# siesta-tool/SequenceDetectionQueryExecutor

Measured on NVIDIA B200. Metric: events scanned/sec (/detection verification), higher is better.
Workload: dtype int32

## Files before the change

sequencedetectionqueryexecutor_b200/csrc/detect.cu:

```cuda
#include <algorithm>
#include <cstdio>
#include <type_traits>
#include <cstdlib>
#include <cstring>
#include <vector>

#include "detect_common.cuh"

namespace siesta {

template <int W, int R, int NF, bool SMEM_RUNS>
struct WarpSmem {
    static constexpr int NE = ROWS_OF(W);
    static constexpr size_t famvv_off = 0;
    static constexpr size_t famvv_bytes = SMEM_RUNS ? sizeof(unsigned long long) * NF * 32 : 0;
    static constexpr size_t rmask_off = famvv_off + famvv_bytes;
    static constexpr size_t rmask_bytes = SMEM_RUNS ? sizeof(typename MaskOps<W>::T) * R * 32 : 0;
    typedef typename std::conditional<W == 1, uint16_t, uint32_t>::type small_t;
    static constexpr size_t small_off = rmask_off + rmask_bytes;
    static constexpr size_t small_bytes = sizeof(small_t) * NE * 32;
    static constexpr size_t rmeta_off = (small_off + small_bytes + 15) & ~(size_t)15;
    static constexpr size_t rmeta_bytes = SMEM_RUNS ? sizeof(uint32_t) * R * 32 : 0;
    static constexpr size_t bytes_off = rmeta_off + rmeta_bytes;
    static constexpr size_t bytes_bytes = SMEM_RUNS ? (size_t)(R + 3 * NF) * 32 : 0;
// ... 775 lines not shown
}

__global__ void set_tail_kernel(int64_t* occ_off, int64_t n_tr, int64_t n_occ, int64_t* ev_off, int64_t n_ev, RebaseOffsets base) {
    occ_off[n_tr] = n_occ + base.occ;
    ev_off[n_occ] = n_ev + base.ev;
}

namespace {

struct DevBuf {
    void* p = nullptr;
    Ctx* c = nullptr;
    explicit DevBuf(Ctx* ctx) : c(ctx) {}
    DevBuf(const DevBuf&) = delete;
    ~DevBuf() { if (p) dev_arena_free(c, p); }
    int alloc(size_t bytes) {
        if (p) { dev_arena_free(c, p); p = nullptr; }
        p = dev_arena_alloc(c, bytes);
        return p ? SIESTA_OK : SIESTA_E_NOMEM;
    }
    template <class T> T* as() const { return reinterpret_cast<T*>(p); }
    void* release() { void* q = p; p = nullptr; return q; }
};

struct View {
    void* p;
    template <class T> T* as() const { return reinterpret_cast<T*>(p); }
};

template <int W, int R, int NF, bool SMEM_RUNS, int MODE>
int launch_detect(const Ctx* ctx, cudaStream_t stream, DetectParams P, const DevNfa& nfa) {
    typedef WarpSmem<W, R, NF, SMEM_RUNS> L;
    const bool needs_aux = MODE == FAST_NK && (P.flags & SIESTA_F_RETURN_ALL) != 0;
    int nt = NT;
    if (const char* env = std::getenv("SIESTA_K1_THREADS")) {
        const int v = std::atoi(env);
        if (v >= 32 && v <= NT_MAX && v % 32 == 0) nt = v;
    }
    const size_t smem = L::total(needs_aux) * (nt / 32);
    auto kern = detect_kernel<W, R, NF, SMEM_RUNS, MODE>;
    SIESTA_CUDA_OK(cudaFuncSetAttribute(kern, cudaFuncAttributeMaxDynamicSharedMemorySize, (int)smem));
    if (const char* env = std::getenv("SIESTA_K1_CARVEOUT")) {
        const int v = std::atoi(env);
        if (v >= 0 && v <= 100) SIESTA_CUDA_OK(cudaFuncSetAttribute(kern, cudaFuncAttributePreferredSharedMemoryCarveout, v));
    }
    int per_sm = 0;
    SIESTA_CUDA_OK(cudaOccupancyMaxActiveBlocksPerMultiprocessor(&per_sm, kern, nt, smem));
    if (per_sm < 1) per_sm = 1;
    const int64_t n_tiles = (P.n_work + 31) / 32;
    const int64_t ctas_needed = (n_tiles + nt / 32 - 1) / (nt / 32);
    if (const char* env = std::getenv("SIESTA_K1_CTAS_PER_SM")) {
        const int v = std::atoi(env);
        if (v >= 1 && v < per_sm) per_sm = v;
    }
    int grid = (int)std::min<int64_t>(ctas_needed, (int64_t)ctx->sm_count * per_sm);
    if (P.n_work_dev) grid = std::min(grid, ctx->sm_count * 2);
    if (grid < 1) grid = 1;
    kern<<<grid, nt, smem, stream>>>(P, nfa);
    SIESTA_LAUNCHED();
    SIESTA_CUDA_OK(cudaGetLastError());
    return SIESTA_OK;
}

}

struct DetectPending {
    Log* log = nullptr;
    cudaStream_t stream = nullptr;
    int64_t n = 0;
    uint32_t flags = 0;
    RebaseOffsets base{0, 0, 0};
    const int64_t* d_cand = nullptr;
    DetectParams P;
    size_t n_blk = 0;
    unsigned long long *d_blk = nullptr, *d_top = nullptr, *d_counters = nullptr;
    int64_t* d_err = nullptr;
    int64_t* d_unsup = nullptr;
    int unsup_slot = 7;
    void* work = nullptr;
    int uniform_k = 0;
    cudaEvent_t ev0 = nullptr, evd = nullptr;
    unsigned long long* h_cnt = nullptr;
    const uint16_t* d_lut = nullptr;
    const uint4* d_nkp_lut = nullptr;
};

static unsigned long long* pinned_counters_get(Ctx* c) {
    std::lock_guard<std::mutex> g(c->arena_mu);
    if (c->pinned_counters.empty()) {
        void* slab = nullptr;
        if (cudaHostAlloc(&slab, 32 * 128, cudaHostAllocDefault) != cudaSuccess) return nullptr;
        c->pinned_slabs.push_back(slab);
        for (int i = 0; i < 32; ++i) c->pinned_counters.push_back(reinterpret_cast<unsigned long long*>(reinterpret_cast<char*>(slab) + 128 * i));
    }
    unsigned long long* p = c->pinned_counters.back();
    c->pinned_counters.pop_back();
    return p;
}
static void pinned_counters_put(Ctx* c, unsigned long long* p) {
    if (!p) return;
    std::lock_guard<std::mutex> g(c->arena_mu);
    c->pinned_counters.push_back(p);
}

static void pending_discard(DetectPending* q) {
    if (!q) return;
    if (q->work) dev_arena_free(q->log->ctx, q->work);
    if (q->ev0) cudaEventDestroy(q->ev0);
    if (q->evd) cudaEventDestroy(q->evd);
    pinned_counters_put(q->log->ctx, q->h_cnt);
    delete q;
}

int detect_device_finish_impl(DetectPending* q, siesta_dev_matches* out);

int detect_device_begin_impl(Log* log, const siesta_nfa* nfa, const int64_t* d_cand, int64_t n_cand, uint32_t flags,
                             cudaStream_t stream, RebaseOffsets base, DetectPending** pending, const DetectPending* sibling) {
    *pending = nullptr;
    base.trace += log->first_trace;
    DevNfa dn;
    int rc = validate_nfa(nfa, flags, &dn);
    if (rc != SIESTA_OK) return rc;
    const Ctx* ctx = log->ctx;
    SIESTA_CUDA_OK(cudaSetDevice(ctx->device));
    if (!stream) stream = ctx->stream;
    const int64_t n = d_cand ? n_cand : log->n_traces;
    const bool return_all = (flags & SIESTA_F_RETURN_ALL) != 0;
    const bool all_cols = (flags & SIESTA_F_NO_EVENT_COLUMNS) == 0;

    std::vector<uint16_t> lut;
    int needs_ts = 0, n_positive = 0;
    build_lut(nfa, dn, log->n_activities, flags, lut, &needs_ts, &n_positive);

    const int64_t wide = std::min<int64_t>(log->n_events, n * 64);
    const int64_t cap_occ = return_all ? wide : n;
    const int64_t cap_ev = (!return_all && !dn.any_kleene) ? n * std::max(1, n_positive) : wide;

    DevBuf work(log->ctx);
    const size_t nn = (size_t)std::max<int64_t>(n, 1);
    size_t w_off = 0;
    auto carve = [&w_off](size_t bytes) {
        const size_t at = w_off;
        w_off += (bytes + 255) & ~(size_t)255;
        return at;
    };
    NkwProgram prog;
    const int nkw_space = nkw_build(dn, flags, &prog);
    std::vector<uint16_t> sigs;
    for (size_t a = 0; a < lut.size(); ++a) {
        const uint16_t sg = lut[a] & 0xFFu;
        if (sg && std::find(sigs.begin(), sigs.end(), sg) == sigs.end()) sigs.push_back(sg);
    }
    const bool use_nkp = nkw_space != NKW_NONE && (!needs_ts || return_all) && log->act_valid && log->n_activities <= 255 && !sigs.empty() && sigs.size() <= 7 &&
                         (reinterpret_cast<uintptr_t>(log->d_act) & 31u) == 0 && std::getenv("SIESTA_K1_NO_NKP") == nullptr;
    const size_t reg2 = use_nkp ? (size_t)std::max<int64_t>(cap_ev, n * (int64_t)std::max(1, n_positive)) : 0;
    const bool use_long = dn.fast_class == FAST_NK && std::getenv("SIESTA_K1_NO_LONG") == nullptr;
    const int64_t cap_long = use_long ? std::min<int64_t>(log->n_events, (int64_t)1 << 21) : 0;
    const size_t long_pool = use_long ? (size_t)std::min<int64_t>(std::max<int64_t>(log->n_events * 64, (int64_t)1 << 20), (int64_t)256 << 20) : 0;
    const size_t n_blk = (nn + GT - 1) / GT;
    const size_t o_ovf2 = use_nkp ? carve(nn * 8) : 0;
    const size_t o_unsup = carve((size_t)SIESTA_MAX_UNSUPPORTED * 8);
    const size_t o_unsup2 = use_long ? carve((size_t)SIESTA_MAX_UNSUPPORTED * 8) : 0;
    const size_t o_pool = carve(long_pool);
    const size_t o_nlut = use_nkp ? carve((size_t)(log->n_activities + 1) * 16) : 0;
    const size_t o_lut = carve(lut.size() * sizeof(uint16_t)), o_nocc = carve(nn * 4), o_stage = carve(nn * 8),
                 o_stage_occ = carve(return_all ? nn * 8 : 0), o_counters = carve(32 * 8), o_err = carve(nn * 8), o_ovf = carve(nn * 8),
                 o_blk = carve(n_blk * 3 * 8), o_top = carve(((n_blk + 1023) / 1024) * 3 * 8), o_occ_nev = carve(return_all ? ((size_t)(cap_occ + cap_long) + (use_nkp ? nn : 0)) * 4 : 0), o_pos = carve(((size_t)cap_ev + reg2 + (size_t)cap_long) * 4);
    size_t o_rank = 0, o_act = 0, o_ts = 0;
    if (all_cols) {
        o_rank = carve(((size_t)cap_ev + reg2 + (size_t)cap_long) * 4);
        o_act = carve(((size_t)cap_ev + reg2 + (size_t)cap_long) * 4);
        o_ts = carve(((size_t)cap_ev + reg2 + (size_t)cap_long) * 8);
    }
    if ((rc = work.alloc(w_off))) return rc;
    char* wb = work.as<char>();
    const View b_lut{wb + o_lut}, b_nocc{wb + o_nocc}, b_stage{wb + o_stage}, b_stage_occ{wb + o_stage_occ},
        b_counters{wb + o_counters}, b_err{wb + o_err}, b_ovf{wb + o_ovf}, b_blk{wb + o_blk}, s_occ_nev{wb + o_occ_nev},
        s_ev_pos{wb + o_pos}, s_ev_rank{all_cols ? wb + o_rank : nullptr}, s_ev_act{all_cols ? wb + o_act : nullptr},
        s_ev_ts{all_cols ? wb + o_ts : nullptr};

    cudaEvent_t ev0 = nullptr, evd = nullptr;
    SIESTA_CUDA_OK(cudaEventCreate(&ev0));
    SIESTA_CUDA_OK(cudaEventCreate(&evd));
    unsigned long long* h_cnt = nullptr;
    const uint4* d_nkp_lut = nullptr;
    struct BeginGuard {
        cudaEvent_t &a, &b;
        unsigned long long*& h;
        Ctx* c;
        bool armed;
        ~BeginGuard() {
            if (!armed) return;
            if (a) cudaEventDestroy(a);
            if (b) cudaEventDestroy(b);
            pinned_counters_put(c, h);
        }
    } begin_guard{ev0, evd, h_cnt, log->ctx, true};
    if (!sibling) SIESTA_CUDA_OK(cudaMemcpyAsync(b_lut.p, lut.data(), lut.size() * sizeof(uint16_t), cudaMemcpyHostToDevice, stream));
    SIESTA_CUDA_OK(cudaMemsetAsync(b_counters.p, 0, 256, stream));
    SIESTA_CUDA_OK(cudaMemsetAsync(b_blk.p, 0, n_blk * 3 * 8, stream));
    SIESTA_CUDA_OK(cudaEventRecord(ev0, stream));

    DetectParams P;
    std::memset(&P, 0, sizeof(P));
    P.trace_off = log->d_trace_off;
    P.act = log->d_act;
    P.ts_ms = log->d_ts_ms;
    P.cand = d_cand;
    P.work = nullptr;
    P.n_work = n;
    P.lut = sibling ? sibling->d_lut : b_lut.as<uint16_t>();
    P.n_act = log->n_activities;
    P.n_events = log->n_events;
    P.alpha_mode = !log->act_valid ? 2 : (log->n_activities <= 32 ? 0 : (log->n_activities <= 64 ? 1 : 2));
    std::memset(P.relrev, 0, sizeof(P.relrev));
    std::memset(P.cls_word, 0, sizeof(P.cls_word));
    std::memset(P.cls_act, 0, sizeof(P.cls_act));
    P.n_planes = 1;
    if (P.alpha_mode != 2) {
        int K = 0;
        for (size_t a = 0; a < lut.size(); ++a) K += lut[a] != 0;
        if (K > 7) P.alpha_mode = 2;
        else {
            int c = 0;
            for (size_t a = 0; a < lut.size(); ++a) {
                if (!lut[a]) continue;
                ++c;
                P.cls_word[c] = lut[a];
                P.cls_act[c] = (int32_t)a;
                for (int p = 0; p < 3; ++p)
                    if ((c >> p) & 1) P.relrev[p][a >> 5] |= 0x80000000u >> (a & 31);
            }
            P.n_planes = K <= 1 ? 1 : (K <= 3 ? 2 : 3);
        }
    }
    P.vec_ok = (reinterpret_cast<uintptr_t>(log->d_act) & 15u) == 0 ? 1 : 0;
    P.flags = flags;
    P.needs_ts = needs_ts;
    P.d_cnt = b_nocc.as<uint32_t>();
    P.d_stage = b_stage.as<int64_t>();
    P.d_stage_occ = b_stage_occ.as<int64_t>();
    P.s_occ_nev = s_occ_nev.as<int32_t>();
    P.s_ev_pos = s_ev_pos.as<int32_t>();
    P.s_ev_rank = s_ev_rank.as<int32_t>();
    P.s_ev_act = s_ev_act.as<int32_t>();
    P.s_ev_ts = s_ev_ts.as<int64_t>();
    P.cap_occ = cap_occ;
    P.cap_ev = cap_ev;
    P.counters = b_counters.as<unsigned long long>();
    P.err_list = b_err.as<int64_t>();
    P.ovf_list = b_ovf.as<int64_t>();
    P.blk_sums = b_blk.as<unsigned long long>();
    P.n_blk = (int64_t)n_blk;

    P.ovf_slot = 4;
    P.tile_slot = 16;
    h_cnt = pinned_counters_get(log->ctx);
    if (!h_cnt) {
        set_error("cudaHostAlloc (counters) failed");
        return SIESTA_E_NOMEM;
    }
    std::memset(h_cnt, 0, 128);
    if (n > 0) {
        if (use_nkp) {
            DetectParams N = P;
            N.ovf_list = reinterpret_cast<int64_t*>(wb + o_ovf2);
            N.ovf_slot = 13;
            N.tile_slot = 18;
            N.fix_ev = cap_ev;
            N.fix_np = std::max(1, n_positive);
            N.fix_occ = return_all ? cap_occ + cap_long : -1;
            std::vector<uint32_t> nlut((size_t)(log->n_activities + 1) * 4, 0u);
            std::memset(N.cls_word, 0, sizeof(N.cls_word));
            for (int a = 0; a <= log->n_activities; ++a) {
                const uint16_t sg = a < log->n_activities ? (lut[a] & 0xFFu) : 0;
                int c = 0;
                if (sg) {
                    c = (int)(std::find(sigs.begin(), sigs.end(), sg) - sigs.begin()) + 1;
                    N.cls_word[c] = sg;
                }
                nlut[4 * a + 0] = (nkw_space == NKW_RAW || c) ? 2u : 1u;
                for (int p = 0; p < 3; ++p) nlut[4 * a + 1 + p] = (c >> p) & 1;
            }
            if (sibling && sibling->d_nkp_lut) N.nkp_lut = sibling->d_nkp_lut;
            else {
                SIESTA_CUDA_OK(cudaMemcpyAsync(wb + o_nlut, nlut.data(), nlut.size() * 4, cudaMemcpyHostToDevice, stream));
                N.nkp_lut = reinterpret_cast<const uint4*>(wb + o_nlut);
            }
            d_nkp_lut = N.nkp_lut;
            N.n_planes = sigs.size() <= 1 ? 1 : (sigs.size() <= 3 ? 2 : 3);
            std::memset(N.st_inv, 0, sizeof(N.st_inv));
            std::memset(N.st_single, 0, sizeof(N.st_single));
            for (int k = 0; k < nfa->n_states; ++k) {
                int n_own = 0, c_own = 0;
                for (int c = 1; c <= (int)sigs.size(); ++c)
                    if (sigs[(size_t)c - 1] & (1u << k)) {
                        ++n_own;
                        c_own = c;
                    }
                if (n_own == 1) {
                    N.st_single[k] = 1;
                    for (int p = 0; p < 3; ++p) N.st_inv[k][p] = ((c_own >> p) & 1) ? 0u : 0xFFFFFFFFu;
                }
            }
            if ((rc = launch_nkp(ctx, stream, N, prog, nkw_space))) return rc;
            P.work = N.ovf_list;
            P.n_work_dev = b_counters.as<unsigned long long>() + 13;
        }
        if (dn.fast_class == FAST_FK2) rc = launch_detect<1, 0, 0, false, FAST_FK2>(ctx, stream, P, dn);
        else if (dn.fast_class == FAST_NK) rc = launch_detect<1, 0, 0, false, FAST_NK>(ctx, stream, P, dn);
        else if (dn.fast_class == FAST_NP1) rc = launch_detect<1, 0, 0, false, FAST_NP1>(ctx, stream, P, dn);
        else rc = launch_detect<1, 16, 16, true, FAST_NONE>(ctx, stream, P, dn);
        if (rc) return rc;
        SIESTA_CUDA_OK(cudaEventRecord(evd, stream));
        DetectParams Q = P;
        Q.work = b_ovf.as<int64_t>();
        Q.n_work_dev = b_counters.as<unsigned long long>() + 4;
        Q.ovf_list = reinterpret_cast<int64_t*>(wb + o_unsup);
        Q.ovf_cap = SIESTA_MAX_UNSUPPORTED;
        Q.ovf_slot = 7;
        Q.tile_slot = 17;
        if (dn.fast_class == FAST_FK2) rc = launch_detect<2, 0, 0, false, FAST_FK2>(ctx, stream, Q, dn);
        else if (dn.fast_class == FAST_NK) rc = launch_detect<2, 0, 0, false, FAST_NK>(ctx, stream, Q, dn);
        else if (dn.fast_class == FAST_NP1) rc = launch_detect<2, 0, 0, false, FAST_NP1>(ctx, stream, Q, dn);
        else rc = launch_detect<2, 1024, 128, false, FAST_NONE>(ctx, stream, Q, dn);
        if (rc) return rc;
        if (use_long) {
            LongParams LQ;
            std::memset(&LQ, 0, sizeof(LQ));
            LQ.work = reinterpret_cast<const int64_t*>(wb + o_unsup);
            LQ.n_work_dev = b_counters.as<unsigned long long>() + 7;
            LQ.work_cap = SIESTA_MAX_UNSUPPORTED;
            LQ.pool = wb + o_pool;
            LQ.pool_bytes = long_pool;
            LQ.ev_base = (int64_t)cap_ev + (int64_t)reg2;
            LQ.ev_cap = cap_long;
            LQ.occ_base = cap_occ;
            LQ.occ_cap = cap_long;
            LQ.unsup = reinterpret_cast<int64_t*>(wb + o_unsup2);
            LQ.unsup_cap = SIESTA_MAX_UNSUPPORTED;
            LQ.n_positive = std::max(1, n_positive);
            detect_long_kernel<<<ctx->sm_count * 2, 128, 0, stream>>>(P, LQ, dn);
            SIESTA_LAUNCHED();
            SIESTA_CUDA_OK(cudaGetLastError());
        }
        if (!sibling) SIESTA_CUDA_OK(cudaMemcpyAsync(h_cnt, b_counters.p, 128, cudaMemcpyDeviceToHost, stream));
    }
    DetectPending* q = new DetectPending();
    q->log = log;
    q->stream = stream;
    q->n = n;
    q->flags = flags;
    q->base = base;
    q->d_cand = d_cand;
    q->P = P;
    q->n_blk = n_blk;
    q->d_blk = b_blk.as<unsigned long long>();
    q->d_top = reinterpret_cast<unsigned long long*>(wb + o_top);
    q->d_counters = b_counters.as<unsigned long long>();
    q->d_err = b_err.as<int64_t>();
    q->d_unsup = reinterpret_cast<int64_t*>(wb + (use_long ? o_unsup2 : o_unsup));
    q->unsup_slot = use_long ? 14 : 7;
    q->work = work.release();
    q->uniform_k = (!return_all && !dn.any_kleene) ? std::max(1, n_positive) : 0;
    q->ev0 = ev0;
    q->evd = evd;
    q->h_cnt = h_cnt;
    q->d_lut = P.lut;
    q->d_nkp_lut = d_nkp_lut;
    begin_guard.armed = false;
    *pending = q;
    return SIESTA_OK;
}

int detect_device_finish_impl(DetectPending* q, siesta_dev_matches* out) {
    std::memset(out, 0, sizeof(*out));
    struct Guard {
        DetectPending* q;
        ~Guard() { pending_discard(q); }
    } guard{q};
    Log* log = q->log;
    const Ctx* ctx = log->ctx;
    SIESTA_CUDA_OK(cudaSetDevice(ctx->device));
    cudaStream_t stream = q->stream;
    const int64_t n = q->n;
    const uint32_t flags = q->flags;
    const bool return_all = (flags & SIESTA_F_RETURN_ALL) != 0;
    const bool all_cols = (flags & SIESTA_F_NO_EVENT_COLUMNS) == 0;
    const RebaseOffsets base = q->base;
    const int64_t* d_cand = q->d_cand;
    const DetectParams& P = q->P;
    const size_t n_blk = q->n_blk;
    unsigned long long* h_cnt = q->h_cnt;
    cudaEvent_t ev0 = q->ev0, evd = q->evd, ev1;
    int rc = SIESTA_OK;
    SIESTA_CUDA_OK(cudaStreamSynchronize(stream));
    if (n > 0) {
        if (h_cnt[7] > SIESTA_MAX_UNSUPPORTED || h_cnt[q->unsup_slot] > SIESTA_MAX_UNSUPPORTED) {
            set_error(std::to_string(h_cnt[7]) + " traces exceed the engine limits (64 pattern-relevant events, 1024 live runs or "
                      "65536 events per trace); at most " + std::to_string(SIESTA_MAX_UNSUPPORTED) + " are listed per request");
            return SIESTA_E_UNSUPPORTED;
        }
        if (h_cnt[5] > 0) {
            set_error("internal: occurrence staging overflow");
            return SIESTA_E_NOMEM;
        }
    }
    SIESTA_CUDA_OK(cudaEventCreate(&ev1));
    struct EvGuard {
        cudaEvent_t e;
        ~EvGuard() { cudaEventDestroy(e); }
    } ev1_guard{ev1};
#ifdef SIESTA_PHASE_TIMING
    fprintf(stderr, "[siesta phase timing] warp-cycles: filter %llu engine %llu output %llu\n", h_cnt[8], h_cnt[9], h_cnt[10]);
#endif
    const int64_t n_occ = (int64_t)h_cnt[0], n_ev = (int64_t)h_cnt[1], n_tr = (int64_t)h_cnt[6], n_err = (int64_t)h_cnt[3];
    const int64_t n_unsup = n > 0 ? (int64_t)h_cnt[q->unsup_slot] : 0;

    DevBuf fin(log->ctx);
    size_t f_off = 0;
    auto fcarve = [&f_off](size_t bytes) {
        const size_t at = f_off;
        f_off += (bytes + 255) & ~(size_t)255;
        return at;
    };
    const size_t q_trace = fcarve((size_t)n_tr * 8), q_occ = fcarve((size_t)(n_tr + 1) * 8), q_evoff = fcarve((size_t)(n_occ + 1) * 8),
                 q_pos = fcarve((size_t)n_ev * 4), q_err = fcarve((size_t)n_err * 8);
    size_t q_rank = 0, q_act = 0, q_ts = 0;
    if (all_cols) {
        q_rank = fcarve((size_t)n_ev * 4);
        q_act = fcarve((size_t)n_ev * 4);
        q_ts = fcarve((size_t)n_ev * 8);
    }
    const size_t q_unsup = fcarve((size_t)n_unsup * 8);
    if ((rc = fin.alloc(f_off))) return rc;
    char* fb = fin.as<char>();
    const View f_unsup{fb + q_unsup};
    const View f_trace{fb + q_trace}, f_occ_off{fb + q_occ}, f_ev_off{fb + q_evoff}, f_pos{fb + q_pos}, f_err{fb + q_err},
        f_rank{all_cols ? fb + q_rank : nullptr}, f_act{all_cols ? fb + q_act : nullptr}, f_ts{all_cols ? fb + q_ts : nullptr};

    if (n > 0) {
        GatherParams G;
        std::memset(&G, 0, sizeof(G));
        G.cand = d_cand;
        G.base = base;
        G.n = n;
        G.d_cnt = P.d_cnt;
        G.d_stage = P.d_stage;
        G.d_stage_occ = return_all ? P.d_stage_occ : nullptr;
        G.n_blk = (int64_t)n_blk;
        G.blk = q->d_blk;
        G.n_chunks = (int64_t)((n_blk + 1023) / 1024);
// ... 467 lines not shown
```

sequencedetectionqueryexecutor_b200/csrc/detect_common.cuh:

```cuda
#pragma once
#include "detect_fast.cuh"

namespace siesta {

constexpr int NT = 128;
constexpr int NT_MAX = 128;
#define ROWS_OF(W) ((W) == 1 ? 24 : 64)

struct DetectParams {
    const int64_t* trace_off;
    const int32_t* act;
    const int64_t* ts_ms;
    const int64_t* cand;
    const int64_t* work;
    int64_t n_work;
    const unsigned long long* n_work_dev;
    int32_t ovf_slot;
    int32_t tile_slot;
    const uint16_t* lut;
    uint32_t relrev[3][2];
    uint16_t cls_word[8];
    int32_t cls_act[8];
    int32_t n_planes;
    int64_t n_events;
    int32_t alpha_mode;
    int32_t vec_ok;
    int32_t n_act;
    uint32_t flags;
    int32_t needs_ts;
    uint32_t* d_cnt;
    int64_t* d_stage;
    int64_t* d_stage_occ;
    int32_t* s_occ_nev;
    int32_t* s_ev_pos;
    int32_t* s_ev_rank;
    int32_t* s_ev_act;
    int64_t* s_ev_ts;
    int64_t cap_occ, cap_ev;
    int64_t fix_ev;
    int32_t fix_np;
    int64_t fix_occ;
    uint32_t st_inv[SIESTA_MAX_STATES][3];
    uint8_t st_single[SIESTA_MAX_STATES];
    const uint4* nkp_lut;
    int32_t tile_batch;
    unsigned long long* counters;
    unsigned long long* blk_sums;
    int64_t n_blk;
    int64_t* err_list;
    int64_t* ovf_list;
    int64_t ovf_cap;
};

__device__ __forceinline__ long long shfl_i64(long long v, int src) {
    int lo = __shfl_sync(0xffffffffu, (int)(v & 0xffffffffll), src);
    int hi = __shfl_sync(0xffffffffu, (int)(v >> 32), src);
    return ((long long)hi << 32) | (unsigned int)lo;
}

enum { ST_NONE = 0, ST_MATCH = 1, ST_ERR = 2, ST_OVF = 3 };

__device__ __forceinline__ void load_sectors(const DetectParams& P, long long e, long long o0, long long o1, int4 (&v)[8]) {
#pragma unroll
    for (int q = 0; q < 4; ++q) {
        const long long c = e + 8 * q;
        if (c >= o1) {
            v[2 * q] = v[2 * q + 1] = make_int4(-1, -1, -1, -1);
        } else if (P.vec_ok && c + 8 <= P.n_events) {
            v[2 * q] = __ldg(reinterpret_cast<const int4*>(P.act + c));
            v[2 * q + 1] = __ldg(reinterpret_cast<const int4*>(P.act + c + 4));
        } else {
            int a[8];
#pragma unroll
            for (int i = 0; i < 8; ++i) a[i] = (c + i < o1 && c + i >= o0) ? __ldg(P.act + c + i) : -1;
            v[2 * q] = make_int4(a[0], a[1], a[2], a[3]);
            v[2 * q + 1] = make_int4(a[4], a[5], a[6], a[7]);
        }
    }
}
__device__ __forceinline__ void load_sectors_vec(const DetectParams& P, long long e, long long o1, int4 (&v)[8]) {
    const int none = P.n_act;
#pragma unroll
    for (int q = 0; q < 4; ++q) {
        const long long c = e + 8 * q;
        if (c >= o1) {
            v[2 * q] = v[2 * q + 1] = make_int4(none, none, none, none);
        } else {
            asm volatile("ld.global.nc.v8.s32 {%0,%1,%2,%3,%4,%5,%6,%7}, [%8];"
                         : "=r"(v[2 * q].x), "=r"(v[2 * q].y), "=r"(v[2 * q].z), "=r"(v[2 * q].w), "=r"(v[2 * q + 1].x),
                           "=r"(v[2 * q + 1].y), "=r"(v[2 * q + 1].z), "=r"(v[2 * q + 1].w)
                         : "l"(P.act + c));
        }
    }
}

__device__ __forceinline__ void load_quarter(const DetectParams& P, long long e, long long o1, int4 (&v)[4]) {
    const int none = P.n_act;
#pragma unroll
    for (int q = 0; q < 2; ++q) {
        const long long c = e + 8 * q;
        if (c >= o1) {
            v[2 * q] = v[2 * q + 1] = make_int4(none, none, none, none);
        } else {
            asm volatile("ld.global.nc.v8.s32 {%0,%1,%2,%3,%4,%5,%6,%7}, [%8];"
                         : "=r"(v[2 * q].x), "=r"(v[2 * q].y), "=r"(v[2 * q].z), "=r"(v[2 * q].w), "=r"(v[2 * q + 1].x),
                           "=r"(v[2 * q + 1].y), "=r"(v[2 * q + 1].z), "=r"(v[2 * q + 1].w)
                         : "l"(P.act + c));
        }
    }
}

__device__ __forceinline__ uint32_t rel_push32(uint32_t pend, uint32_t relrev, int a) {
    uint32_t t;
    asm("shl.b32 %0, %1, %2;" : "=r"(t) : "r"(relrev), "r"(a));
    return __funnelshift_r(t, pend, 31);
}
__device__ __forceinline__ uint32_t rel_push64(uint32_t pend, uint32_t relrev_a, uint32_t relrev_b, int a) {
    uint32_t t;
    const uint32_t w = ((unsigned)a < 32u) ? relrev_a : (((unsigned)a < 64u) ? relrev_b : 0u);
    asm("shl.b32 %0, %1, %2;" : "=r"(t) : "r"(w), "r"(a & 31));
    return __funnelshift_r(t, pend, 31);
}

template <int NPL, bool WIDE>
__device__ __forceinline__ void scan_block(const DetectParams& P, const int4 (&v)[8], uint32_t (&pl)[3]) {
#pragma unroll
    for (int q = 7; q >= 0; --q) {
        const int a[4] = {v[q].x, v[q].y, v[q].z, v[q].w};
#pragma unroll
        for (int i = 3; i >= 0; --i) {
#pragma unroll
            for (int p = 0; p < NPL; ++p)
                pl[p] = WIDE ? rel_push64(pl[p], P.relrev[p][0], P.relrev[p][1], a[i]) : rel_push32(pl[p], P.relrev[p][0], a[i]);
        }
    }
}

__device__ __forceinline__ int rel_seconds(long long diff_ms) {
    if ((unsigned long long)diff_ms < (1ull << 32)) return (int)((uint32_t)diff_ms / 1000u);
    return (int)(diff_ms / 1000);
}

__device__ __forceinline__ void cp_async8(void* smem_dst, const void* gsrc) {
    const uint32_t d = (uint32_t)__cvta_generic_to_shared(smem_dst);
    asm volatile("cp.async.ca.shared.global [%0], [%1], 8;" ::"r"(d), "l"(gsrc) : "memory");
}
__device__ __forceinline__ void cp_async4(void* smem_dst, const void* gsrc) {
    const uint32_t d = (uint32_t)__cvta_generic_to_shared(smem_dst);
    asm volatile("cp.async.ca.shared.global [%0], [%1], 4;" ::"r"(d), "l"(gsrc) : "memory");
}
__device__ __forceinline__ void cp_async_wait_all() { asm volatile("cp.async.wait_all;" ::: "memory"); }


int launch_nkp(const Ctx* ctx, cudaStream_t stream, const DetectParams& P, const NkwProgram& prog, int space);

}
```

sequencedetectionqueryexecutor_b200/csrc/detect_nkp.cu:

```cuda
#include "detect_common.cuh"

namespace siesta {

#ifndef SIESTA_NKP_MIN_CTAS
#define SIESTA_NKP_MIN_CTAS 8
#endif
#ifndef SIESTA_NKP_PREFETCH
#define SIESTA_NKP_PREFETCH 0
#endif

constexpr int LUT_SKEW = 8;
template <int NPL, bool RAW>
__device__ __forceinline__ void scan16(const uint4* __restrict__ lut, const int4 (&v)[4], uint32_t (&pl)[3], uint32_t& racc) {
#pragma unroll
    for (int q = 3; q >= 0; --q) {
        const int a[4] = {v[q].x, v[q].y, v[q].z, v[q].w};
#pragma unroll
        for (int i = 3; i >= 0; --i) {
            const uint4 w = lut[a[i] * LUT_SKEW];
            pl[0] = pl[0] * w.x + w.y;
            if (NPL > 1) pl[1] = pl[1] * w.x + w.z;
            if (NPL > 2) pl[2] = pl[2] * w.x + w.w;
            if (!RAW) racc = racc * 2u + w.x;
        }
    }
}

__device__ __forceinline__ int select32(uint32_t x, int r) {
    int pos = 0;
#pragma unroll
    for (int w = 16; w >= 1; w >>= 1) {
        const int c = __popc((x >> pos) & ((1u << w) - 1u));
        if (r >= c) {
            r -= c;
            pos += w;
        }
    }
    return pos;
}
__device__ __forceinline__ int select64(unsigned long long x, int r) {
    const uint32_t lo = (uint32_t)x, hi = (uint32_t)(x >> 32);
    const int c = __popc(lo);
    return r >= c ? 32 + select32(hi, r - c) : select32(lo, r);
}

template <int NPL, bool RAW, bool MARKOV>
__global__ void __launch_bounds__(NT_MAX, SIESTA_NKP_MIN_CTAS) detect_nkp_kernel(const __grid_constant__ DetectParams P, const __grid_constant__ NkwProgram prog) {
    typedef typename std::conditional<RAW, unsigned long long, uint32_t>::type mask_t;
    typedef unsigned long long u64;
    typedef NkwBits<mask_t> B;
    const int lane = threadIdx.x & 31;
    extern __shared__ uint4 s_lut_all[];
    for (int i = threadIdx.x; i < (P.n_act + 1) * LUT_SKEW; i += blockDim.x) s_lut_all[i] = P.nkp_lut[i / LUT_SKEW];
    __syncthreads();
    const uint4* s_lut = s_lut_all + (lane & (LUT_SKEW - 1));
    const bool evt_pos = (P.flags & SIESTA_F_EVT_POS) != 0;
    const bool all_cols = (P.flags & SIESTA_F_NO_EVENT_COLUMNS) == 0;
    const bool return_all = (P.flags & SIESTA_F_RETURN_ALL) != 0;
    const bool first_only = (P.flags & (SIESTA_F_COUNT_MATCHES | SIESTA_F_RETURN_ALL)) == 0;

    const long long n_work = P.n_work_dev ? (long long)__ldg(P.n_work_dev) : (long long)P.n_work;
    const long long n_tiles = (n_work + 31) / 32;
    const int batch = P.tile_batch;
    long long tile = 0, next_batch = 0, next_batch2 = 0;
    if (lane == 0) {
        tile = (long long)atomicAdd(P.counters + P.tile_slot, (unsigned long long)batch);
        next_batch = (long long)atomicAdd(P.counters + P.tile_slot, (unsigned long long)batch);
    }
    tile = shfl_i64(tile, 0);
    int left = batch;
    unsigned long long acc_occ = 0, acc_ev = 0, acc_emit = 0;

    auto locate = [&](long long tl, int64_t& ci_, long long& o0_, long long& o1_) {
        const int64_t wi = tl * 32 + lane;
        ci_ = -1;
        o0_ = o1_ = 0;
        if (tl < n_tiles && wi < n_work) {
            ci_ = P.work ? P.work[wi] : wi;
            const int64_t t = P.cand ? P.cand[ci_] : ci_;
            o0_ = P.trace_off[t];
            o1_ = P.trace_off[t + 1];
        }
    };
    int64_t ci;
    long long o0, o1;
    locate(tile, ci, o0, o1);
    while (tile < n_tiles) {
        if (left == batch && lane == 0) next_batch2 = (long long)atomicAdd(P.counters + P.tile_slot, (unsigned long long)batch);
        const long long nxt = left > 1 ? tile + 1 : shfl_i64(next_batch, 0);
#if SIESTA_NKP_PREFETCH
        int64_t nci;
        long long no0, no1;
        locate(nxt, nci, no0, no1);
#endif

        const long long e0 = o0 & ~7LL;
        const int lead = (int)(o0 - e0);
        const long long span = (o1 - o0) + lead;
        bool fits = span <= 64 && ((o1 + 7) & ~7LL) <= P.n_events;
        const long long o1s = fits ? o1 : e0;
        u64 valid = 0;
        if (fits && o1 > o0) valid = (span == 64 ? ~0ull : ((1ull << (int)span) - 1ull)) & ~((1ull << lead) - 1ull);
        const bool second = __any_sync(0xffffffffu, fits && span > 32);

        uint32_t q[3] = {0u, 0u, 0u}, qb[3] = {0u, 0u, 0u}, ra = 0u, rb = 0u;
        {
            int4 A[4], B[4];
            if (second) {
                load_quarter(P, e0 + 48, o1s, A);
                load_quarter(P, e0 + 32, o1s, B);
                scan16<NPL, RAW>(s_lut, A, RAW ? qb : q, rb);
                load_quarter(P, e0 + 16, o1s, A);
                scan16<NPL, RAW>(s_lut, B, RAW ? qb : q, rb);
                load_quarter(P, e0, o1s, B);
                rb += 1u;
            } else {
                load_quarter(P, e0 + 16, o1s, A);
                load_quarter(P, e0, o1s, B);
            }
            scan16<NPL, RAW>(s_lut, A, q, ra);
            scan16<NPL, RAW>(s_lut, B, q, ra);
            ra += 1u;
        }
        mask_t pl[3];
        u64 Rv;
        if constexpr (RAW) {
#pragma unroll
            for (int p = 0; p < 3; ++p) pl[p] = p < NPL ? (((u64)q[p] | ((u64)qb[p] << 32)) & valid) : 0ull;
            Rv = pl[0] | pl[1] | pl[2];
        } else {
            const u64 Rraw = (u64)ra | ((u64)rb << 32);
            Rv = Rraw & valid;
            const int n_lead = __popc(ra & ((1u << lead) - 1u));
            const int n_valid = __popcll(Rv);
            if (n_lead + n_valid > 32) fits = false;
            const uint32_t keep = B::one_shl(n_valid) - 1u;
#pragma unroll
            for (int p = 0; p < 3; ++p) pl[p] = p < NPL ? ((q[p] >> n_lead) & keep) : 0u;
        }
        mask_t T[SIESTA_MAX_STATES + 1];
#pragma unroll
        for (int k = 0; k <= SIESTA_MAX_STATES; ++k) {
            T[k] = 0;
            if (k < SIESTA_MAX_STATES && k < prog.n_states) {
                if (P.st_single[k]) {
                    mask_t m = ~(mask_t)0;
#pragma unroll
                    for (int p = 0; p < NPL; ++p) m &= pl[p] ^ (mask_t)(long long)(int)P.st_inv[k][p];
                    T[k] = m;
                } else {
#pragma unroll
                    for (int c = 1; c < (1 << NPL); ++c)
                        if (P.cls_word[c] & (1u << k)) {
                            mask_t m = ~(mask_t)0;
#pragma unroll
                            for (int p = 0; p < NPL; ++p) m &= ((c >> p) & 1) ? pl[p] : ~pl[p];
                            T[k] |= m;
                        }
                }
            }
        }

        int status = ST_NONE;
        unsigned n_emitted = 0;
        mask_t best = 0;
        if (ci >= 0 && o1 > o0) {
            if (!fits) status = ST_OVF;
            else if (Rv) {
                bool hit;
                if constexpr (MARKOV) hit = nkw_eval_markov<mask_t>(prog, T, best, n_emitted);
                else hit = nkw_eval<mask_t>(prog, T, best, n_emitted, first_only);
                if (hit) status = (return_all && n_emitted > 1) ? ST_OVF : ST_MATCH;
            }
        }

        const unsigned my_occ = status == ST_MATCH ? 1u : 0u;
        const unsigned my_ev = status == ST_MATCH ? (unsigned)B::popc(best) : 0u;
        unsigned i1 = my_ev;
        unsigned long long i2 = (status == ST_MATCH) ? n_emitted : 0u;
#pragma unroll
        for (int d = 1; d < 32; d <<= 1) {
            const unsigned y1 = __shfl_up_sync(0xffffffffu, i1, d);
            if (lane >= d) i1 += y1;
        }
        if (!first_only) {
#pragma unroll
            for (int d = 1; d < 32; d <<= 1) {
                const unsigned long long y2 = __shfl_up_sync(0xffffffffu, i2, d);
                if (lane >= d) i2 += y2;
            }
        }
        const unsigned n_match = __popc(__ballot_sync(0xffffffffu, status == ST_MATCH));
        acc_occ += n_match;
        acc_ev += i1;
        acc_emit += i2;
        const unsigned tot1 = __shfl_sync(0xffffffffu, i1, 31);
        if (lane == 31 && n_match) {
            unsigned long long* b = P.blk_sums + (tile >> 3);
            atomicAdd(b, (unsigned long long)n_match);
            atomicAdd(b + P.n_blk, (unsigned long long)n_match);
            atomicAdd(b + 2 * P.n_blk, (unsigned long long)i1);
        }
        const long long base1 = P.fix_ev + tile * 32 * P.fix_np;
        if (ci >= 0) {
            P.d_cnt[ci] = my_occ | (my_ev << 16);
            if (status == ST_MATCH) {
                P.d_stage[ci] = base1 + (long long)(i1 - my_ev);
                if (P.fix_occ >= 0) {
                    P.d_stage_occ[ci] = P.fix_occ + ci;
                    P.s_occ_nev[P.fix_occ + ci] = (int32_t)my_ev;
                }
            } else if (status == ST_OVF) {
                const unsigned long long at = atomicAdd(P.counters + P.ovf_slot, 1ull);
                P.ovf_list[at] = ci;
            }
        }
        if (tot1 > 0) {
            for (unsigned f0 = 0; f0 < tot1; f0 += 32) {
                const unsigned f = f0 + lane;
                int lo = 0, hi = 31;
#pragma unroll
                for (int it = 0; it < 5; ++it) {
                    const int mid = (lo + hi) >> 1;
                    const unsigned vmid = __shfl_sync(0xffffffffu, i1, mid);
                    if (vmid > f) hi = mid; else lo = mid + 1;
                }
                const int owner = lo & 31;
                const unsigned o_incl = __shfl_sync(0xffffffffu, i1, owner);
                const unsigned o_ev = __shfl_sync(0xffffffffu, my_ev, owner);
                mask_t m;
                if constexpr (RAW) m = (mask_t)shfl_i64((long long)best, owner);
                else m = __shfl_sync(0xffffffffu, best, owner);
                const u64 o_R = (u64)shfl_i64((long long)Rv, owner);
                const long long o_o0 = shfl_i64(o0, owner);
                if (f < tot1) {
                    int k = (int)(f - (o_incl - o_ev));
                    for (; k > 0; --k) m &= m - 1;
                    int j, rank;
                    if constexpr (RAW) {
                        j = __ffsll((long long)m) - 1;
                        rank = __popcll(o_R & ((1ull << j) - 1ull));
                    } else {
                        rank = __ffs((int)m) - 1;
                        j = select64(o_R, rank);
                    }
                    const int src = j - (int)(o_o0 & 7);
                    const long long at = base1 + f;
                    P.s_ev_pos[at] = src;
                    if (all_cols) {
                        const long long* tsp = reinterpret_cast<const long long*>(P.ts_ms) + o_o0;
                        const int32_t c_act = __ldg(P.act + o_o0 + src);
                        const long long raw = __ldg(tsp + src);
                        const long long o_t0 = evt_pos ? 0 : __ldg(tsp + (__ffsll((long long)o_R) - 1 - (int)(o_o0 & 7)));
                        P.s_ev_rank[at] = rank;
                        P.s_ev_act[at] = c_act;
                        P.s_ev_ts[at] = evt_pos ? raw : (long long)rel_seconds(raw - o_t0) * 1000 + o_t0;
                    }
                }
            }
        }
        tile = nxt;
        if (--left == 0) {
            left = batch;
            next_batch = next_batch2;
        }
#if SIESTA_NKP_PREFETCH
        ci = nci;
        o0 = no0;
        o1 = no1;
#else
        locate(tile, ci, o0, o1);
#endif
    }
    if (lane == 31) {
        if (acc_occ) {
            atomicAdd(P.counters + 0, acc_occ);
            atomicAdd(P.counters + 6, acc_occ);
        }
        if (acc_ev) atomicAdd(P.counters + 1, acc_ev);
        if (acc_emit) atomicAdd(P.counters + 2, acc_emit);
    }
}

namespace {
template <int NPL, bool RAW, bool MARKOV>
int launch_one(const Ctx* ctx, cudaStream_t stream, DetectParams P, const NkwProgram& prog) {
    auto kern = detect_nkp_kernel<NPL, RAW, MARKOV>;
    const size_t smem = (size_t)(P.n_act + 1) * LUT_SKEW * sizeof(uint4);
    int per_sm = 0;
    SIESTA_CUDA_OK(cudaOccupancyMaxActiveBlocksPerMultiprocessor(&per_sm, kern, NT, smem));
    if (per_sm < 1) per_sm = 1;
    if (const char* env = std::getenv("SIESTA_K1_CTAS_PER_SM")) {
        const int v = std::atoi(env);
        if (v >= 1 && v < per_sm) per_sm = v;
    }
    if (const char* env = std::getenv("SIESTA_NKP_CARVEOUT")) {
        const int v = std::atoi(env);
        if (v >= 0 && v <= 100) SIESTA_CUDA_OK(cudaFuncSetAttribute(kern, cudaFuncAttributePreferredSharedMemoryCarveout, v));
    }
    const int64_t n_tiles = (P.n_work + 31) / 32;
    const int64_t ctas_needed = (n_tiles + NT / 32 - 1) / (NT / 32);
    int grid = (int)std::min<int64_t>(ctas_needed, (int64_t)ctx->sm_count * per_sm);
    if (grid < 1) grid = 1;
    const int64_t per_warp = n_tiles / ((int64_t)grid * (NT / 32));
    P.tile_batch = per_warp >= 64 ? 4 : (per_warp >= 16 ? 2 : 1);
    if (const char* env = std::getenv("SIESTA_NKP_TILE_BATCH")) {
        const int v = std::atoi(env);
        if (v >= 1 && v <= 64) P.tile_batch = v;
    }
    kern<<<grid, NT, smem, stream>>>(P, prog);
    SIESTA_LAUNCHED();
    SIESTA_CUDA_OK(cudaGetLastError());
    return SIESTA_OK;
}
}

int launch_nkp(const Ctx* ctx, cudaStream_t stream, const DetectParams& P, const NkwProgram& prog, int space) {
    const bool raw = space == NKW_RAW;
    const bool markov = prog.markov && std::getenv("SIESTA_NKP_NO_MARKOV") == nullptr;
#define SIESTA_NKP_GO(NPL)                                                                                              \
    (raw ? (markov ? launch_one<NPL, true, true>(ctx, stream, P, prog) : launch_one<NPL, true, false>(ctx, stream, P, prog))   \
         : (markov ? launch_one<NPL, false, true>(ctx, stream, P, prog) : launch_one<NPL, false, false>(ctx, stream, P, prog)))
    if (P.n_planes == 1) return SIESTA_NKP_GO(1);
    if (P.n_planes == 2) return SIESTA_NKP_GO(2);
    return SIESTA_NKP_GO(3);
#undef SIESTA_NKP_GO
}

}
```

Baseline: 551.5 billion.

## Split NKP detection into a coalesced plane-building scan kernel plus detect pass

Adds a separate scan kernel that turns each trace's activity ids into per-class bit planes. It reads trace events warp-cooperatively with coalesced loads, classifies them through a byte code table in shared memory, and transposes through shared-memory rows. The planes are stored in global scratch. The detect kernel now streams these precomputed planes instead of doing per-thread vector loads and multiply-add lookups into a skewed uint4 LUT. The aim is to replace uncoalesced per-lane sector loads and LUT bank pressure with coalesced access, at the cost of an extra launch and a global round-trip of plane data.

```diff
diff --git a/sequencedetectionqueryexecutor_b200/csrc/detect.cu b/sequencedetectionqueryexecutor_b200/csrc/detect.cu
--- a/sequencedetectionqueryexecutor_b200/csrc/detect.cu
+++ b/sequencedetectionqueryexecutor_b200/csrc/detect.cu
@@ -881,7 +881,7 @@
     cudaEvent_t ev0 = nullptr, evd = nullptr;
     unsigned long long* h_cnt = nullptr;
     const uint16_t* d_lut = nullptr;
-    const uint4* d_nkp_lut = nullptr;
+    const uint8_t* d_nkp_code = nullptr;
 };
 
 static unsigned long long* pinned_counters_get(Ctx* c) {
@@ -961,7 +961,10 @@
     const size_t o_unsup = carve((size_t)SIESTA_MAX_UNSUPPORTED * 8);
     const size_t o_unsup2 = use_long ? carve((size_t)SIESTA_MAX_UNSUPPORTED * 8) : 0;
     const size_t o_pool = carve(long_pool);
-    const size_t o_nlut = use_nkp ? carve((size_t)(log->n_activities + 1) * 16) : 0;
+    const size_t o_ncode = use_nkp ? carve((size_t)log->n_activities + 1) : 0;
+    const int nkp_planes = sigs.size() <= 1 ? 1 : (sigs.size() <= 3 ? 2 : 3);
+    const size_t o_pl64 = use_nkp ? carve(nn * 8 * (nkw_space == NKW_RAW ? nkp_planes : 1)) : 0;
+    const size_t o_pl32 = use_nkp && nkw_space != NKW_RAW ? carve(nn * 4 * nkp_planes) : 0;
     const size_t o_lut = carve(lut.size() * sizeof(uint16_t)), o_nocc = carve(nn * 4), o_stage = carve(nn * 8),
                  o_stage_occ = carve(return_all ? nn * 8 : 0), o_counters = carve(32 * 8), o_err = carve(nn * 8), o_ovf = carve(nn * 8),
                  o_blk = carve(n_blk * 3 * 8), o_top = carve(((n_blk + 1023) / 1024) * 3 * 8), o_occ_nev = carve(return_all ? ((size_t)(cap_occ + cap_long) + (use_nkp ? nn : 0)) * 4 : 0), o_pos = carve(((size_t)cap_ev + reg2 + (size_t)cap_long) * 4);
@@ -982,7 +985,7 @@
     SIESTA_CUDA_OK(cudaEventCreate(&ev0));
     SIESTA_CUDA_OK(cudaEventCreate(&evd));
     unsigned long long* h_cnt = nullptr;
-    const uint4* d_nkp_lut = nullptr;
+    const uint8_t* d_nkp_code = nullptr;
     struct BeginGuard {
         cudaEvent_t &a, &b;
         unsigned long long*& h;
@@ -1069,7 +1072,7 @@
             N.fix_ev = cap_ev;
             N.fix_np = std::max(1, n_positive);
             N.fix_occ = return_all ? cap_occ + cap_long : -1;
-            std::vector<uint32_t> nlut((size_t)(log->n_activities + 1) * 4, 0u);
+            std::vector<uint8_t> ncode((size_t)log->n_activities + 1, 0u);
             std::memset(N.cls_word, 0, sizeof(N.cls_word));
             for (int a = 0; a <= log->n_activities; ++a) {
                 const uint16_t sg = a < log->n_activities ? (lut[a] & 0xFFu) : 0;
@@ -1078,16 +1081,18 @@
                     c = (int)(std::find(sigs.begin(), sigs.end(), sg) - sigs.begin()) + 1;
                     N.cls_word[c] = sg;
                 }
-                nlut[4 * a + 0] = (nkw_space == NKW_RAW || c) ? 2u : 1u;
-                for (int p = 0; p < 3; ++p) nlut[4 * a + 1 + p] = (c >> p) & 1;
-            }
-            if (sibling && sibling->d_nkp_lut) N.nkp_lut = sibling->d_nkp_lut;
+                ncode[(size_t)a] = (uint8_t)c;
+            }
+            if (sibling && sibling->d_nkp_code) N.nkp_code = sibling->d_nkp_code;
             else {
-                SIESTA_CUDA_OK(cudaMemcpyAsync(wb + o_nlut, nlut.data(), nlut.size() * 4, cudaMemcpyHostToDevice, stream));
-                N.nkp_lut = reinterpret_cast<const uint4*>(wb + o_nlut);
-            }
-            d_nkp_lut = N.nkp_lut;
-            N.n_planes = sigs.size() <= 1 ? 1 : (sigs.size() <= 3 ? 2 : 3);
+                SIESTA_CUDA_OK(cudaMemcpyAsync(wb + o_ncode, ncode.data(), ncode.size(), cudaMemcpyHostToDevice, stream));
+                N.nkp_code = reinterpret_cast<const uint8_t*>(wb + o_ncode);
+            }
+            d_nkp_code = N.nkp_code;
+            N.n_planes = nkp_planes;
+            N.pl64 = reinterpret_cast<unsigned long long*>(wb + o_pl64);
+            N.pl32 = reinterpret_cast<uint32_t*>(wb + o_pl32);
+            N.pl_ld = (int64_t)nn;
             std::memset(N.st_inv, 0, sizeof(N.st_inv));
             std::memset(N.st_single, 0, sizeof(N.st_single));
             for (int k = 0; k < nfa->n_states; ++k) {
@@ -1166,7 +1171,7 @@
     q->evd = evd;
     q->h_cnt = h_cnt;
     q->d_lut = P.lut;
-    q->d_nkp_lut = d_nkp_lut;
+    q->d_nkp_code = d_nkp_code;
     begin_guard.armed = false;
     *pending = q;
     return SIESTA_OK;
diff --git a/sequencedetectionqueryexecutor_b200/csrc/detect_common.cuh b/sequencedetectionqueryexecutor_b200/csrc/detect_common.cuh
--- a/sequencedetectionqueryexecutor_b200/csrc/detect_common.cuh
+++ b/sequencedetectionqueryexecutor_b200/csrc/detect_common.cuh
@@ -42,7 +42,10 @@
     int64_t fix_occ;
     uint32_t st_inv[SIESTA_MAX_STATES][3];
     uint8_t st_single[SIESTA_MAX_STATES];
-    const uint4* nkp_lut;
+    const uint8_t* nkp_code;
+    unsigned long long* pl64;
+    uint32_t* pl32;
+    int64_t pl_ld;
     int32_t tile_batch;
     unsigned long long* counters;
     unsigned long long* blk_sums;
@@ -78,38 +81,6 @@
         }
     }
 }
-__device__ __forceinline__ void load_sectors_vec(const DetectParams& P, long long e, long long o1, int4 (&v)[8]) {
-    const int none = P.n_act;
-#pragma unroll
-    for (int q = 0; q < 4; ++q) {
-        const long long c = e + 8 * q;
-        if (c >= o1) {
-            v[2 * q] = v[2 * q + 1] = make_int4(none, none, none, none);
-        } else {
-            asm volatile("ld.global.nc.v8.s32 {%0,%1,%2,%3,%4,%5,%6,%7}, [%8];"
-                         : "=r"(v[2 * q].x), "=r"(v[2 * q].y), "=r"(v[2 * q].z), "=r"(v[2 * q].w), "=r"(v[2 * q + 1].x),
-                           "=r"(v[2 * q + 1].y), "=r"(v[2 * q + 1].z), "=r"(v[2 * q + 1].w)
-                         : "l"(P.act + c));
-        }
-    }
-}
-
-__device__ __forceinline__ void load_quarter(const DetectParams& P, long long e, long long o1, int4 (&v)[4]) {
-    const int none = P.n_act;
-#pragma unroll
-    for (int q = 0; q < 2; ++q) {
-        const long long c = e + 8 * q;
-        if (c >= o1) {
-            v[2 * q] = v[2 * q + 1] = make_int4(none, none, none, none);
-        } else {
-            asm volatile("ld.global.nc.v8.s32 {%0,%1,%2,%3,%4,%5,%6,%7}, [%8];"
-                         : "=r"(v[2 * q].x), "=r"(v[2 * q].y), "=r"(v[2 * q].z), "=r"(v[2 * q].w), "=r"(v[2 * q + 1].x),
-                           "=r"(v[2 * q + 1].y), "=r"(v[2 * q + 1].z), "=r"(v[2 * q + 1].w)
-                         : "l"(P.act + c));
-        }
-    }
-}
-
 __device__ __forceinline__ uint32_t rel_push32(uint32_t pend, uint32_t relrev, int a) {
     uint32_t t;
     asm("shl.b32 %0, %1, %2;" : "=r"(t) : "r"(relrev), "r"(a));
diff --git a/sequencedetectionqueryexecutor_b200/csrc/detect_nkp.cu b/sequencedetectionqueryexecutor_b200/csrc/detect_nkp.cu
--- a/sequencedetectionqueryexecutor_b200/csrc/detect_nkp.cu
+++ b/sequencedetectionqueryexecutor_b200/csrc/detect_nkp.cu
@@ -5,26 +5,6 @@
 #ifndef SIESTA_NKP_MIN_CTAS
 #define SIESTA_NKP_MIN_CTAS 8
 #endif
-#ifndef SIESTA_NKP_PREFETCH
-#define SIESTA_NKP_PREFETCH 0
-#endif
-
-constexpr int LUT_SKEW = 8;
-template <int NPL, bool RAW>
-__device__ __forceinline__ void scan16(const uint4* __restrict__ lut, const int4 (&v)[4], uint32_t (&pl)[3], uint32_t& racc) {
-#pragma unroll
-    for (int q = 3; q >= 0; --q) {
-        const int a[4] = {v[q].x, v[q].y, v[q].z, v[q].w};
-#pragma unroll
-        for (int i = 3; i >= 0; --i) {
-            const uint4 w = lut[a[i] * LUT_SKEW];
-            pl[0] = pl[0] * w.x + w.y;
-            if (NPL > 1) pl[1] = pl[1] * w.x + w.z;
-            if (NPL > 2) pl[2] = pl[2] * w.x + w.w;
-            if (!RAW) racc = racc * 2u + w.x;
-        }
-    }
-}
 
 __device__ __forceinline__ int select32(uint32_t x, int r) {
     int pos = 0;
@@ -42,6 +22,105 @@
     const uint32_t lo = (uint32_t)x, hi = (uint32_t)(x >> 32);
     const int c = __popc(lo);
     return r >= c ? 32 + select32(hi, r - c) : select32(lo, r);
+}
+
+constexpr int SCAN_ROW = 80;
+
+__device__ __forceinline__ uint32_t gather4(uint32_t w, int p) { return ((w & (0x01010101u << p)) * (0x10204080u >> p)) >> 28; }
+
+template <int NPL>
+__device__ __forceinline__ void planes32(const uint4 (&c)[2], uint32_t (&pl)[3]) {
+    const uint32_t w[8] = {c[0].x, c[0].y, c[0].z, c[0].w, c[1].x, c[1].y, c[1].z, c[1].w};
+#pragma unroll
+    for (int p = 0; p < NPL; ++p) {
+        uint32_t v = 0;
+#pragma unroll
+        for (int k = 0; k < 8; ++k) v |= gather4(w[k], p) << (4 * k);
+        pl[p] = v;
+    }
+}
+
+template <int NPL, bool RAW>
+__global__ void __launch_bounds__(NT, 8) nkp_scan_kernel(const __grid_constant__ DetectParams P) {
+    const int lane = threadIdx.x & 31;
+    __shared__ uint8_t s_code[256];
+    __shared__ __align__(16) uint8_t s_rows[NT / 32][32 * SCAN_ROW];
+    for (int a = threadIdx.x; a <= P.n_act; a += blockDim.x) s_code[a] = P.nkp_code[a];
+    __syncthreads();
+    uint8_t* rows = s_rows[threadIdx.x >> 5];
+    uint4* my_row = reinterpret_cast<uint4*>(rows + lane * SCAN_ROW);
+    const int none = P.n_act;
+    const uint32_t lt = (1u << lane) - 1u;
+
+    const long long n_work = P.n_work_dev ? (long long)__ldg(P.n_work_dev) : (long long)P.n_work;
+    const long long n_tiles = (n_work + 31) / 32;
+    const long long warps = (long long)gridDim.x * (NT / 32);
+    for (long long tile = (long long)blockIdx.x * (NT / 32) + (threadIdx.x >> 5); tile < n_tiles; tile += warps) {
+        const long long wi = tile * 32 + lane;
+        long long o0 = 0, o1 = 0;
+        if (wi < n_work) {
+            const int64_t ci = P.work ? P.work[wi] : wi;
+            const int64_t t = P.cand ? P.cand[ci] : ci;
+            o0 = P.trace_off[t];
+            o1 = P.trace_off[t + 1];
+        }
+        const int len = o1 - o0 <= 64 ? (int)(o1 - o0) : 0;
+        const bool second = __any_sync(0xffffffffu, len > 32);
+        if (!RAW) {
+            my_row[0] = my_row[1] = make_uint4(0u, 0u, 0u, 0u);
+            __syncwarp();
+        }
+
+        unsigned long long R = 0;
+#pragma unroll 1
+        for (int s0 = 0; s0 < 32; s0 += 8) {
+            int a[8], b[8];
+#pragma unroll
+            for (int k = 0; k < 8; ++k) {
+                const int ls = __shfl_sync(0xffffffffu, len, s0 + k);
+                const int* src = P.act + shfl_i64(o0, s0 + k);
+                a[k] = lane < ls ? __ldg(src + lane) : none;
+                b[k] = second && 32 + lane < ls ? __ldg(src + 32 + lane) : none;
+            }
+#pragma unroll
+            for (int k = 0; k < 8; ++k) {
+                uint8_t* row = rows + (s0 + k) * SCAN_ROW;
+                const uint8_t ca = s_code[a[k]], cb = s_code[b[k]];
+                if constexpr (RAW) {
+                    row[lane] = ca;
+                    if (second) row[32 + lane] = cb;
+                } else {
+                    const uint32_t ba = __ballot_sync(0xffffffffu, ca != 0), bb = __ballot_sync(0xffffffffu, cb != 0);
+                    if (ca) row[__popc(ba & lt)] = ca;
+                    if (cb) row[__popc(ba) + __popc(bb & lt)] = cb;
+                    if (lane == s0 + k) R = (unsigned long long)ba | ((unsigned long long)bb << 32);
+                }
+            }
+        }
+        __syncwarp();
+
+        uint32_t q[3] = {0u, 0u, 0u}, qb[3] = {0u, 0u, 0u};
+        {
+            const uint4 c[2] = {my_row[0], my_row[1]};
+            planes32<NPL>(c, q);
+        }
+        if (RAW && second) {
+            const uint4 c[2] = {my_row[2], my_row[3]};
+            planes32<NPL>(c, qb);
+        }
+        __syncwarp();
+
+        if (wi < n_work) {
+            if constexpr (RAW) {
+#pragma unroll
+                for (int p = 0; p < NPL; ++p) P.pl64[p * P.pl_ld + wi] = (unsigned long long)q[p] | ((unsigned long long)qb[p] << 32);
+            } else {
+                P.pl64[wi] = R;
+#pragma unroll
+                for (int p = 0; p < NPL; ++p) P.pl32[p * P.pl_ld + wi] = q[p];
+            }
+        }
+    }
 }
 
 template <int NPL, bool RAW, bool MARKOV>
@@ -50,10 +129,6 @@
     typedef unsigned long long u64;
     typedef NkwBits<mask_t> B;
     const int lane = threadIdx.x & 31;
-    extern __shared__ uint4 s_lut_all[];
-    for (int i = threadIdx.x; i < (P.n_act + 1) * LUT_SKEW; i += blockDim.x) s_lut_all[i] = P.nkp_lut[i / LUT_SKEW];
-    __syncthreads();
-    const uint4* s_lut = s_lut_all + (lane & (LUT_SKEW - 1));
     const bool evt_pos = (P.flags & SIESTA_F_EVT_POS) != 0;
     const bool all_cols = (P.flags & SIESTA_F_NO_EVENT_COLUMNS) == 0;
     const bool return_all = (P.flags & SIESTA_F_RETURN_ALL) != 0;
@@ -88,55 +163,20 @@
     while (tile < n_tiles) {
         if (left == batch && lane == 0) next_batch2 = (long long)atomicAdd(P.counters + P.tile_slot, (unsigned long long)batch);
         const long long nxt = left > 1 ? tile + 1 : shfl_i64(next_batch, 0);
-#if SIESTA_NKP_PREFETCH
-        int64_t nci;
-        long long no0, no1;
-        locate(nxt, nci, no0, no1);
-#endif
-
-        const long long e0 = o0 & ~7LL;
-        const int lead = (int)(o0 - e0);
-        const long long span = (o1 - o0) + lead;
-        bool fits = span <= 64 && ((o1 + 7) & ~7LL) <= P.n_events;
-        const long long o1s = fits ? o1 : e0;
-        u64 valid = 0;
-        if (fits && o1 > o0) valid = (span == 64 ? ~0ull : ((1ull << (int)span) - 1ull)) & ~((1ull << lead) - 1ull);
-        const bool second = __any_sync(0xffffffffu, fits && span > 32);
-
-        uint32_t q[3] = {0u, 0u, 0u}, qb[3] = {0u, 0u, 0u}, ra = 0u, rb = 0u;
-        {
-            int4 A[4], B[4];
-            if (second) {
-                load_quarter(P, e0 + 48, o1s, A);
-                load_quarter(P, e0 + 32, o1s, B);
-                scan16<NPL, RAW>(s_lut, A, RAW ? qb : q, rb);
-                load_quarter(P, e0 + 16, o1s, A);
-                scan16<NPL, RAW>(s_lut, B, RAW ? qb : q, rb);
-                load_quarter(P, e0, o1s, B);
-                rb += 1u;
+        const int64_t wi = tile * 32 + lane;
+        bool fits = o1 - o0 <= 64;
+        mask_t pl[3] = {0, 0, 0};
+        u64 Rv = 0;
+        if (ci >= 0) {
+            if constexpr (RAW) {
+#pragma unroll
+                for (int p = 0; p < NPL; ++p) Rv |= pl[p] = __ldcs(P.pl64 + p * P.pl_ld + wi);
             } else {
-                load_quarter(P, e0 + 16, o1s, A);
-                load_quarter(P, e0, o1s, B);
-            }
-            scan16<NPL, RAW>(s_lut, A, q, ra);
-            scan16<NPL, RAW>(s_lut, B, q, ra);
-            ra += 1u;
-        }
-        mask_t pl[3];
-        u64 Rv;
-        if constexpr (RAW) {
-#pragma unroll
-            for (int p = 0; p < 3; ++p) pl[p] = p < NPL ? (((u64)q[p] | ((u64)qb[p] << 32)) & valid) : 0ull;
-            Rv = pl[0] | pl[1] | pl[2];
-        } else {
-            const u64 Rraw = (u64)ra | ((u64)rb << 32);
-            Rv = Rraw & valid;
-            const int n_lead = __popc(ra & ((1u << lead) - 1u));
-            const int n_valid = __popcll(Rv);
-            if (n_lead + n_valid > 32) fits = false;
-            const uint32_t keep = B::one_shl(n_valid) - 1u;
-#pragma unroll
-            for (int p = 0; p < 3; ++p) pl[p] = p < NPL ? ((q[p] >> n_lead) & keep) : 0u;
+                Rv = __ldcs(P.pl64 + wi);
+                if (__popcll(Rv) > 32) fits = false;
+#pragma unroll
+                for (int p = 0; p < NPL; ++p) pl[p] = __ldcs(P.pl32 + p * P.pl_ld + wi);
+            }
         }
         mask_t T[SIESTA_MAX_STATES + 1];
 #pragma unroll
@@ -244,14 +284,13 @@
                         rank = __ffs((int)m) - 1;
                         j = select64(o_R, rank);
                     }
-                    const int src = j - (int)(o_o0 & 7);
                     const long long at = base1 + f;
-                    P.s_ev_pos[at] = src;
+                    P.s_ev_pos[at] = j;
                     if (all_cols) {
                         const long long* tsp = reinterpret_cast<const long long*>(P.ts_ms) + o_o0;
-                        const int32_t c_act = __ldg(P.act + o_o0 + src);
-                        const long long raw = __ldg(tsp + src);
-                        const long long o_t0 = evt_pos ? 0 : __ldg(tsp + (__ffsll((long long)o_R) - 1 - (int)(o_o0 & 7)));
+                        const int32_t c_act = __ldg(P.act + o_o0 + j);
+                        const long long raw = __ldg(tsp + j);
+                        const long long o_t0 = evt_pos ? 0 : __ldg(tsp + (__ffsll((long long)o_R) - 1));
                         P.s_ev_rank[at] = rank;
                         P.s_ev_act[at] = c_act;
                         P.s_ev_ts[at] = evt_pos ? raw : (long long)rel_seconds(raw - o_t0) * 1000 + o_t0;
@@ -264,13 +303,7 @@
             left = batch;
             next_batch = next_batch2;
         }
-#if SIESTA_NKP_PREFETCH
-        ci = nci;
-        o0 = no0;
-        o1 = no1;
-#else
         locate(tile, ci, o0, o1);
-#endif
     }
     if (lane == 31) {
         if (acc_occ) {
@@ -285,18 +318,23 @@
 namespace {
 template <int NPL, bool RAW, bool MARKOV>
 int launch_one(const Ctx* ctx, cudaStream_t stream, DetectParams P, const NkwProgram& prog) {
+    {
+        auto scan = nkp_scan_kernel<NPL, RAW>;
+        int per_sm = 0;
+        SIESTA_CUDA_OK(cudaOccupancyMaxActiveBlocksPerMultiprocessor(&per_sm, scan, NT, 0));
+        const int64_t ctas_needed = ((P.n_work + 31) / 32 + NT / 32 - 1) / (NT / 32);
+        const int grid = (int)std::max<int64_t>(1, std::min<int64_t>(ctas_needed, (int64_t)ctx->sm_count * std::max(per_sm, 1)));
+        scan<<<grid, NT, 0, stream>>>(P);
+        SIESTA_LAUNCHED();
+        SIESTA_CUDA_OK(cudaGetLastError());
+    }
     auto kern = detect_nkp_kernel<NPL, RAW, MARKOV>;
-    const size_t smem = (size_t)(P.n_act + 1) * LUT_SKEW * sizeof(uint4);
     int per_sm = 0;
-    SIESTA_CUDA_OK(cudaOccupancyMaxActiveBlocksPerMultiprocessor(&per_sm, kern, NT, smem));
+    SIESTA_CUDA_OK(cudaOccupancyMaxActiveBlocksPerMultiprocessor(&per_sm, kern, NT, 0));
     if (per_sm < 1) per_sm = 1;
     if (const char* env = std::getenv("SIESTA_K1_CTAS_PER_SM")) {
         const int v = std::atoi(env);
         if (v >= 1 && v < per_sm) per_sm = v;
-    }
-    if (const char* env = std::getenv("SIESTA_NKP_CARVEOUT")) {
-        const int v = std::atoi(env);
-        if (v >= 0 && v <= 100) SIESTA_CUDA_OK(cudaFuncSetAttribute(kern, cudaFuncAttributePreferredSharedMemoryCarveout, v));
     }
     const int64_t n_tiles = (P.n_work + 31) / 32;
     const int64_t ctas_needed = (n_tiles + NT / 32 - 1) / (NT / 32);
@@ -308,7 +346,7 @@
         const int v = std::atoi(env);
         if (v >= 1 && v <= 64) P.tile_batch = v;
     }
-    kern<<<grid, NT, smem, stream>>>(P, prog);
+    kern<<<grid, NT, 0, stream>>>(P, prog);
     SIESTA_LAUNCHED();
     SIESTA_CUDA_OK(cudaGetLastError());
     return SIESTA_OK;
```

New measurement: 411.6 billion, median of 6. 0.746x the previous value.
